# uthree/tinyvc

Measured on AMD Instinct MI355X. Metric: audio-samples/sec (16 kHz) end-to-end VC, higher is better.
Workload: dtype f32 (fp32 in / out / accumulate; channel contractions as two-term fp16 splits on v_mfma_f32_32x32x16_f16: 22-bit significands, three part-products per fp32 product)

## Files before the change

tinyvc_amd/csrc/knn.hip:

```cpp
#include "knn_blob.h"
#include "knn_search.h"
#include "split_fp16.h"
#include "tvc_common.h"

namespace tvc {

constexpr int KNN_BLOCKS = 1024;

constexpr int QN_WAVES = 16;
static __global__ __launch_bounds__(QN_WAVES * 64) void query_normalize_kernel(const float* __restrict__ src, float* __restrict__ qn, int B, int Bsrc, int T,
                                                                     uint4* __restrict__ qh, int* __restrict__ cnt, int* __restrict__ flag,
                                                                     const KnnSegs segs, int* __restrict__ col2seg) {
    __shared__ float part[QN_WAVES][64];
    const int lane = threadIdx.x & 63, wave = threadIdx.x >> 6;
    const long ncols = (long)B * T;
    long n, nn;
    bool ok;
    int sg;
    if (qh) {
        const int tile = blockIdx.x >> 2;
        sg = seg_find<3>(segs, tile);
        const KnnSeg g = seg_get(segs, sg);
        const long loc = (long)(tile - g.u[3]) * 256 + (blockIdx.x & 3) * 64 + lane;
        ok = loc < g.ncols;
        n = g.col0 + loc;
        nn = ok ? n : g.col0 + g.ncols - 1;
    } else {
        n = blockIdx.x * 64L + lane;
        ok = n < ncols;
        nn = ok ? n : ncols - 1;
        sg = col2seg ? seg_find<4>(segs, (int)nn) : 0;
    }
    if (blockIdx.x == 0 && flag)
        for (int i = threadIdx.x; i < segs.n; i += QN_WAVES * 64) flag[i] = 0;
    if (wave == 0 && ok && cnt) cnt[n] = 0;
    if (wave == 0 && ok && col2seg) col2seg[n] = sg;
    const int b = (int)(nn / T), t = (int)(nn - (long)b * T);
    const float* p = src + (long)(b % Bsrc) * KD * T + t;
    float* q = qn + (long)b * KD * T + t;
    constexpr int KW = KD / QN_WAVES;
    const int k0 = wave * KW;
    float x[KW];
#pragma unroll
    for (int i = 0; i < KW; ++i) x[i] = p[(long)(k0 + i) * T];
    float s = 0.f;
#pragma unroll
    for (int i = 0; i < KW; ++i) s = fmaf(x[i], x[i], s);
    part[wave][lane] = s;
    __syncthreads();
    float ss = part[0][lane];
#pragma unroll
    for (int w = 1; w < QN_WAVES; ++w) ss += part[w][lane];
    const float den = sqrtf(ss) + 1e-6f;
    uint4* qhp = qh ? qh + (blockIdx.x >> 2) * (long)(STEPS * 2 * 256) + (blockIdx.x & 3) * 64 + lane : nullptr;
#pragma unroll
    for (int i = 0; i < KW; i += 8) {
        const int k = k0 + i;
        float v[8];
#pragma unroll
        for (int j = 0; j < 8; ++j) v[j] = ok ? x[i + j] / den : 0.f;
        if (ok) {
#pragma unroll
            for (int j = 0; j < 8; ++j) q[(long)(k + j) * T] = v[j];
        }
        if (qh) {
            unsigned o[4];
#pragma unroll
            for (int j = 0; j < 4; ++j) {
                const __half2 h = __floats2half2_rn(v[2 * j], v[2 * j + 1]);
                o[j] = (unsigned)__half_as_ushort(__low2half(h)) | ((unsigned)__half_as_ushort(__high2half(h)) << 16);
            }
            qhp[(long)(k >> 3) * 256] = make_uint4(o[0], o[1], o[2], o[3]);
        }
    }
}

typedef __bf16 bf16x8 __attribute__((ext_vector_type(8)));
typedef __bf16 bf16x2 __attribute__((ext_vector_type(2)));
__device__ __forceinline__ void split8_bf3(const float (&v)[8], uint4& p1, uint4& p2, uint4& p3) {
    unsigned o1[4], o2[4], o3[4];
#pragma unroll
    for (int j = 0; j < 4; ++j) {
        f32x2 a = {v[2 * j], v[2 * j + 1]};
        bf16x2 h1 = __builtin_convertvector(a, bf16x2);
        f32x2 r = a - __builtin_convertvector(h1, f32x2);
        bf16x2 h2 = __builtin_convertvector(r, bf16x2);
        f32x2 r2 = r - __builtin_convertvector(h2, f32x2);
        bf16x2 h3 = __builtin_convertvector(r2, bf16x2);
        o1[j] = __builtin_bit_cast(unsigned, h1);
        o2[j] = __builtin_bit_cast(unsigned, h2);
        o3[j] = __builtin_bit_cast(unsigned, h3);
    }
    p1 = make_uint4(o1[0], o1[1], o1[2], o1[3]);
    p2 = make_uint4(o2[0], o2[1], o2[2], o2[3]);
    p3 = make_uint4(o3[0], o3[1], o3[2], o3[3]);
}
__device__ __forceinline__ void split8_half(const u32x4 h8, uint4& p1, uint4& p2) {
    const f16x8 hv = __builtin_bit_cast(f16x8, h8);
    unsigned o1[4], o2[4];
#pragma unroll
    for (int j = 0; j < 4; ++j) {
        f32x2 a = {(float)hv[2 * j], (float)hv[2 * j + 1]};
        bf16x2 h1 = __builtin_convertvector(a, bf16x2);
        f32x2 r = a - __builtin_convertvector(h1, f32x2);
        bf16x2 h2 = __builtin_convertvector(r, bf16x2);
        o1[j] = __builtin_bit_cast(unsigned, h1);
        o2[j] = __builtin_bit_cast(unsigned, h2);
    }
    p1 = make_uint4(o1[0], o1[1], o1[2], o1[3]);
    p2 = make_uint4(o2[0], o2[1], o2[2], o2[3]);
}

constexpr int KNN_QT = 256;
constexpr int KNN_A_U4 = 12 * 64, KNN_X_U4 = 3 * 2 * KNN_QT;
template <bool F16>
__device__ __forceinline__ void knn_topk_body(const float* __restrict__ blob, long Npad, int N, const float* __restrict__ qn, int ncols, int col0, int cstride,
                                              int T, int unit, int nsplit, int tiles_per_split, float* __restrict__ cand_v, int* __restrict__ cand_i,
                                              uint4* smem) {
    constexpr int NP = F16 ? 2 : 3;
    constexpr int GP = F16 ? 4 : 12;
    uint4* As = smem;
    uint4* Xs = smem + 2 * KNN_A_U4;
    const uint4* img = F16 ? blob_img16(blob, KIND_F16, N, Npad) : blob_img3(blob, N);
    const float* inv = blob_inv(blob, KIND_F16, N, Npad);

    const int tid = threadIdx.x, lane = tid & 63, wave = tid >> 6;
    const int wm = wave >> 2, wn = wave & 3;
    const int l31 = lane & 31, lh = lane >> 5;
    const int split = unit % nsplit;
    const int qtile = unit / nsplit;
    const int n0 = qtile * KNN_QT;
    const int mtiles = (int)(Npad >> 7);
    const int mt_lo = split * tiles_per_split;
    const int mt_hi = min(mtiles, mt_lo + tiles_per_split);
    const int G = (mt_hi - mt_lo) * STEPS;

    const float* qp;
    int xdst;
    {
        const int g = tid >> 8, pos = tid & 255;
        int n = n0 + pos;
        n = col0 + (n < ncols ? n : ncols - 1);
        const int b = n / T, t = n - b * T;
        qp = qn + ((long)b * KD + 8 * g) * T + t;
        xdst = g * KNN_QT + pos;
    }
    const bool a2 = !F16 && wave < 4;
    const bool a1 = !F16 || wave < 4;
    float xr[8];
    u32x4 ar[2];
    auto gload = [&](int g) __attribute__((always_inline)) {
        const int mt = mt_lo + g / STEPS, st = g - (g / STEPS) * STEPS;
        const uint4* src = img + ((long)mt * STEPS + st) * (GP * 64) + lane;
        if (a1) ar[0] = *reinterpret_cast<const u32x4*>(src + wave * 64);
        if (a2) ar[1] = *reinterpret_cast<const u32x4*>(src + (wave + 8) * 64);
#pragma unroll
        for (int j = 0; j < 8; ++j) xr[j] = qp[(long)(st * 16 + j) * T];
    };
    auto lstore = [&](int buf) __attribute__((always_inline)) {
        uint4* ab = As + buf * KNN_A_U4;
        if (F16) {
            if (a1) {
                uint4 p1, p2;
                split8_half(ar[0], p1, p2);
                ab[(wave * 2) * 64 + lane] = p1;
                ab[(wave * 2 + 1) * 64 + lane] = p2;
            }
        } else {
            *reinterpret_cast<u32x4*>(ab + wave * 64 + lane) = ar[0];
            if (a2) *reinterpret_cast<u32x4*>(ab + (wave + 8) * 64 + lane) = ar[1];
        }
        uint4 p1, p2, p3;
        split8_bf3(xr, p1, p2, p3);
        uint4* xb = Xs + buf * KNN_X_U4;
        xb[xdst] = p1;
        xb[2 * KNN_QT + xdst] = p2;
        xb[4 * KNN_QT + xdst] = p3;
    };

    Top4 top[2];
    top[0].init();
    top[1].init();
    f32x16 acc[2][2];
#pragma unroll
    for (int i = 0; i < 2; ++i)
#pragma unroll
        for (int j = 0; j < 2; ++j)
#pragma unroll
            for (int r = 0; r < 16; ++r) acc[i][j][r] = 0.f;

    if (G > 0) {
        gload(0);
        lstore(0);
        if (G > 1) gload(1);
        slab_barrier();
    }
    for (int g = 0; g < G; ++g) {
        const int cur = g & 1;
        if (g + 1 < G) {
            lstore(cur ^ 1);
            if (g + 2 < G) gload(g + 2);
        }
        const uint4* as = As + cur * KNN_A_U4 + wm * (2 * NP * 64) + lane;
        const uint4* xs = Xs + cur * KNN_X_U4 + lh * KNN_QT + wn * 64 + l31;
        bf16x8 af[2][NP], bf[2][3];
#pragma unroll
        for (int j = 0; j < 2; ++j)
#pragma unroll
            for (int p = 0; p < 3; ++p) bf[j][p] = __builtin_bit_cast(bf16x8, xs[p * 2 * KNN_QT + j * 32]);
#pragma unroll
        for (int i = 0; i < 2; ++i)
#pragma unroll
            for (int p = 0; p < NP; ++p) af[i][p] = __builtin_bit_cast(bf16x8, as[(i * NP + p) * 64]);
        constexpr int NQ = F16 ? 5 : 6;
        constexpr int PA3[6] = {2, 1, 0, 1, 0, 0}, PB3[6] = {0, 1, 2, 0, 1, 0};
        constexpr int PA2[5] = {1, 0, 1, 0, 0}, PB2[5] = {1, 2, 0, 1, 0};
#pragma unroll
        for (int q = 0; q < NQ; ++q)
#pragma unroll
            for (int i = 0; i < 2; ++i)
#pragma unroll
                for (int j = 0; j < 2; ++j)
                    acc[i][j] = __builtin_amdgcn_mfma_f32_32x32x16_bf16(af[i][F16 ? PA2[q < 5 ? q : 0] : PA3[q]], bf[j][F16 ? PB2[q < 5 ? q : 0] : PB3[q]],
                                                                        acc[i][j], 0, 0, 0);
        const int st = g - (g / STEPS) * STEPS;
        if (st == STEPS - 1) {
            const int m0 = (mt_lo + g / STEPS) * 128;
#pragma unroll
            for (int i = 0; i < 2; ++i)
#pragma unroll
                for (int r = 0; r < 16; ++r) {
                    const int row = m0 + (wm * 2 + i) * 32 + (r & 3) + 8 * (r >> 2) + 4 * lh;
                    if (row < N) {
                        const float sc = F16 ? inv[row] : 1.f;
#pragma unroll
                        for (int j = 0; j < 2; ++j) top[j].insert(nan_max(F16 ? acc[i][j][r] * sc : acc[i][j][r]), row);
                    }
#pragma unroll
                    for (int j = 0; j < 2; ++j) acc[i][j][r] = 0.f;
                }
        }
        slab_barrier();
    }

    float (*mv)[16] = reinterpret_cast<float (*)[16]>(smem);
    int (*mi)[16] = reinterpret_cast<int (*)[16]>(reinterpret_cast<float*>(smem) + KNN_QT * 16);
#pragma unroll
    for (int j = 0; j < 2; ++j) {
        const int q = wn * 64 + j * 32 + l31;
        const int slot = (wm * 2 + lh) * 4;
#pragma unroll
        for (int e = 0; e < 4; ++e) {
            mv[q][slot + e] = top[j].v[e];
            mi[q][slot + e] = top[j].i[e];
        }
    }
    __syncthreads();
    if (tid < KNN_QT) {
        Top4 t4;
        t4.init();
        for (int e = 0; e < 16; ++e) t4.insert(mv[tid][e], mi[tid][e]);
        int n = n0 + tid;
        if (n < ncols) {
            long o = ((long)split * cstride + col0 + n) * 4;
#pragma unroll
            for (int e = 0; e < 4; ++e) {
                cand_v[o + e] = t4.v[e];
                cand_i[o + e] = t4.i[e];
            }
        }
    }
}

static __global__ __launch_bounds__(512) void knn_topk_split_kernel(const KnnSegs segs, const float* __restrict__ qn, int cstride, int T,
                                                                    float* __restrict__ cand_v, int* __restrict__ cand_i,
                                                                    const int* __restrict__ flags) {
    __shared__ __attribute__((aligned(16))) uint4 smem[2 * (KNN_A_U4 + KNN_X_U4)];
    const int si = seg_find<2>(segs, blockIdx.x);
    const KnnSeg g = seg_get(segs, si);
    if (g.two && flags[si] == 0) return;
    const int kind = blob_kind(g.blob);
    const int unit = blockIdx.x - g.u[2];
    if (kind == KIND_F16) knn_topk_body<true>(g.blob, blob_npad(g.N), g.N, qn, g.ncols, g.col0, cstride, T, unit, g.nsE, g.tpsE, cand_v, cand_i, smem);
    else knn_topk_body<false>(g.blob, blob_npad(g.N), g.N, qn, g.ncols, g.col0, cstride, T, unit, g.nsE, g.tpsE, cand_v, cand_i, smem);
}

constexpr int C_QT = 256, C_MT = 256, C_K = 64, C_STEPS = KD / C_K;
constexpr int C_A_U4 = 4 * 8 * 64, C_X_U4 = 4 * 2 * C_QT;
constexpr int C_LDS = 2 * (C_A_U4 + C_X_U4) * 16;
constexpr int C_CAP = 256;
constexpr float C_EPS = 1.25e-3f;
constexpr int KNN_COARSE_MIN = 4096;

struct Top4V {
    float v[4];
    __device__ __forceinline__ void init() { v[0] = v[1] = v[2] = v[3] = -INFINITY; }
    __device__ __forceinline__ void insert(float x) {
        if (!(x > v[3])) return;
        if (x > v[0]) { v[3] = v[2]; v[2] = v[1]; v[1] = v[0]; v[0] = x; }
        else if (x > v[1]) { v[3] = v[2]; v[2] = v[1]; v[1] = x; }
        else if (x > v[2]) { v[3] = v[2]; v[2] = x; }
        else v[3] = x;
    }
};

template <bool F16, int MODE>
static __device__ __forceinline__ void knn_coarse_body(const float* __restrict__ blob, long Npad, int N, const uint4* __restrict__ qh,
                                                       int ncols, int cstride, int unit, int nsplit, int tiles_per_split, int t2_cover,
                                                       float* __restrict__ c4v, int ns_sample,
                                                       int* __restrict__ cnt, int* __restrict__ cand, float* __restrict__ candv,
                                                       int* __restrict__ overflow) {
    extern __shared__ __attribute__((aligned(16))) uint4 csmem[];
    uint4* As = csmem;
    uint4* Xs = csmem + 2 * C_A_U4;
    const int kind = F16 ? KIND_F16 : KIND_F32;
    const uint4* img = blob_img16(blob, kind, N, Npad);
    const float* inv = blob_inv(blob, kind, N, Npad);

    const int tid = threadIdx.x, lane = tid & 63, wave = tid >> 6;
    const int wm = wave >> 2, wn = wave & 3;
    const int l31 = lane & 31, lh = lane >> 5;
    const int split = unit % nsplit;
    const int qtile = unit / nsplit;
    const int n0 = qtile * C_QT;
    const int mtiles = (int)(Npad >> 7);
    const int t_lo = split * tiles_per_split;
    const int t_hi = min(t2_cover, t_lo + tiles_per_split);
    const int G = (t_hi - t_lo) * C_STEPS;

    const uint4* xsrc = qh + (long)qtile * (STEPS * 2 * 256) + (tid & 511);
    u32x4 ar[4], xr[4];
    auto gload = [&](int g) __attribute__((always_inline)) {
        const int t2 = t_lo + g / C_STEPS, st = g - (g / C_STEPS) * C_STEPS;
#pragma unroll
        for (int i = 0; i < 4; ++i) {
            const int piece = wave + 8 * i, k16 = piece >> 3, mt8 = piece & 7;
            int t128 = 2 * t2 + (mt8 >> 2);
            t128 = t128 < mtiles ? t128 : mtiles - 1;
            ar[i] = *reinterpret_cast<const u32x4*>(img + (((long)t128 * STEPS + 4 * st + k16) * 4 + (mt8 & 3)) * 64 + lane);
            xr[i] = *reinterpret_cast<const u32x4*>(xsrc + (long)(4 * st + i) * 512);
        }
    };
    auto lstore = [&](int buf) __attribute__((always_inline)) {
#pragma unroll
        for (int i = 0; i < 4; ++i) {
            *reinterpret_cast<u32x4*>(As + buf * C_A_U4 + tid + 512 * i) = ar[i];
            *reinterpret_cast<u32x4*>(Xs + buf * C_X_U4 + tid + 512 * i) = xr[i];
        }
    };

    Top4V top[2];
    top[0].init();
    top[1].init();
    float th[2] = {INFINITY, INFINITY};
    if (MODE == 1) {
#pragma unroll
        for (int j = 0; j < 2; ++j) {
            const int n = n0 + wn * 64 + j * 32 + l31;
            if (n < ncols) {
                Top4V t4;
                t4.init();
                for (int sp = 0; sp < ns_sample; ++sp) {
                    const float4 v4 = *reinterpret_cast<const float4*>(c4v + ((long)sp * cstride + n) * 4);
                    t4.insert(v4.x);
                    t4.insert(v4.y);
                    t4.insert(v4.z);
                    t4.insert(v4.w);
                }
                th[j] = t4.v[3] - 2.f * C_EPS;
            }
        }
    }
    f32x16 acc[4][2];
#pragma unroll
    for (int i = 0; i < 4; ++i)
#pragma unroll
        for (int j = 0; j < 2; ++j)
#pragma unroll
            for (int r = 0; r < 16; ++r) acc[i][j][r] = 0.f;

    if (G > 0) {
        gload(0);
        lstore(0);
        gload(G > 1 ? 1 : 0);
        slab_barrier();
    }
    for (int g = 0; g < G; ++g) {
        const int cur = g & 1;
        lstore(cur ^ 1);
        gload(g + 2 < G ? g + 2 : G - 1);
        const uint4* as = As + cur * C_A_U4 + wm * (4 * 64) + lane;
        const uint4* xs = Xs + cur * C_X_U4 + lh * C_QT + wn * 64 + l31;
#pragma unroll
        for (int k16 = 0; k16 < 4; ++k16) {
            f16x8 af[4], bf[2];
#pragma unroll
            for (int i = 0; i < 4; ++i) af[i] = __builtin_bit_cast(f16x8, as[(k16 * 8 + i) * 64]);
#pragma unroll
            for (int j = 0; j < 2; ++j) bf[j] = __builtin_bit_cast(f16x8, xs[k16 * 2 * C_QT + j * 32]);
#pragma unroll
            for (int i = 0; i < 4; ++i)
#pragma unroll
                for (int j = 0; j < 2; ++j) acc[i][j] = __builtin_amdgcn_mfma_f32_32x32x16_f16(af[i], bf[j], acc[i][j], 0, 0, 0);
        }
        const int st = g - (g / C_STEPS) * C_STEPS;
        if (st == C_STEPS - 1) {
            const int t2 = t_lo + g / C_STEPS;
            const int m0 = t2 * C_MT;
            float imx = 1.f;
            if (F16) {
                const float* im = blob_invmax(blob, Npad);
                const int ta = 2 * t2 < mtiles ? 2 * t2 : mtiles - 1, tb = 2 * t2 + 1 < mtiles ? 2 * t2 + 1 : mtiles - 1;
                imx = fmaxf(im[ta], im[tb]);
            }
            const bool whole = m0 + C_MT <= N;
#pragma unroll
            for (int i = 0; i < 4; ++i)
#pragma unroll
                for (int j = 0; j < 2; ++j) {
                    float mx = acc[i][j][0];
                    bool anynan = false;
#pragma unroll
                    for (int r = 1; r < 16; ++r) mx = fmaxf(mx, acc[i][j][r]);
#pragma unroll
                    for (int r = 0; r < 16; ++r) anynan |= acc[i][j][r] != acc[i][j][r];
                    bool maybe;
                    if (MODE == 0) maybe = anynan || !((F16 ? fmaxf(mx, 0.f) * imx : mx) <= top[j].v[3]);
                    else maybe = anynan || (F16 ? fmaxf(mx, 0.f) * imx : mx) >= th[j];
                    if (__builtin_amdgcn_ballot_w64(maybe) != 0ull) {
#pragma unroll
                        for (int r = 0; r < 16; ++r) {
                            const int row = m0 + (wm * 4 + i) * 32 + (r & 3) + 8 * (r >> 2) + 4 * lh;
                            if (whole || row < N) {
                                const float a = acc[i][j][r];
                                if (MODE == 0) {
                                    if (!F16) {
                                        top[j].insert(nan_max(a));
                                    } else if (!(fmaxf(a, 0.f) * imx <= top[j].v[3])) {
                                        top[j].insert(nan_max(a * inv[row]));
                                    }
                                } else {
                                    bool hit;
                                    float cv = a;
                                    if (!F16) hit = !(a < th[j]);
                                    else {
                                        hit = a != a || (fmaxf(a, 0.f) * imx >= th[j]);
                                        if (hit) {
                                            cv = a * inv[row];
                                            hit = a != a || cv >= th[j];
                                        }
                                    }
                                    hit = hit && th[j] != INFINITY;
                                    if (hit) {
                                        const int n = n0 + wn * 64 + j * 32 + l31;
                                        const int pos = atomicAdd(&cnt[n], 1);
                                        if (pos < C_CAP) {
                                            cand[(long)n * C_CAP + pos] = row;
                                            candv[(long)n * C_CAP + pos] = cv;
                                        } else *overflow = 1;
                                    }
                                }
                            }
                        }
                    }
#pragma unroll
                    for (int r = 0; r < 16; ++r) acc[i][j][r] = 0.f;
                }
        }
        slab_barrier();
    }
    if (MODE == 1) return;

    float (*mv)[16] = reinterpret_cast<float (*)[16]>(csmem);
#pragma unroll
    for (int j = 0; j < 2; ++j) {
        const int q = wn * 64 + j * 32 + l31;
        const int slot = (wm * 2 + lh) * 4;
#pragma unroll
        for (int e = 0; e < 4; ++e) mv[q][slot + e] = top[j].v[e];
    }
    __syncthreads();
    if (tid < C_QT) {
        Top4V t4;
        t4.init();
        for (int e = 0; e < 16; ++e) t4.insert(mv[tid][e]);
        const int n = n0 + tid;
        if (n < ncols) {
            const long o = ((long)split * cstride + n) * 4;
#pragma unroll
            for (int e = 0; e < 4; ++e) c4v[o + e] = t4.v[e];
        }
    }
}

template <int MODE>
static __global__ __launch_bounds__(512) void knn_coarse_kernel(const KnnSegs segs, const uint4* __restrict__ qh, int cstride,
                                                                float* __restrict__ c4v, int* __restrict__ cnt, int* __restrict__ cand,
                                                                float* __restrict__ candv, int* __restrict__ flags) {
    const int si = seg_find<MODE>(segs, blockIdx.x);
    const KnnSeg g = seg_get(segs, si);
    const int unit = blockIdx.x - g.u[MODE];
    const int nsplit = MODE ? g.nsB : g.nsA, tps = MODE ? g.tpsB : g.tpsA, cover = MODE ? g.t2 : g.sample;
    const uint4* q = qh + (long)g.u[3] * (STEPS * 2 * 256);
    float* c4 = c4v + (long)g.col0 * 4;
    int* ct = cnt + g.col0;
    int* cd = cand + (long)g.col0 * C_CAP;
    float* cdv = candv + (long)g.col0 * C_CAP;
    if (blob_kind(g.blob) == KIND_F16)
        knn_coarse_body<true, MODE>(g.blob, blob_npad(g.N), g.N, q, g.ncols, cstride, unit, nsplit, tps, cover, c4, g.nsA, ct, cd, cdv, flags + si);
    else
        knn_coarse_body<false, MODE>(g.blob, blob_npad(g.N), g.N, q, g.ncols, cstride, unit, nsplit, tps, cover, c4, g.nsA, ct, cd, cdv, flags + si);
}

static __global__ __launch_bounds__(256) void knn_rescore_kernel(const KnnSegs segs, const int* __restrict__ col2seg, const float* __restrict__ qn,
                                                                 int ncols, int T, const int* __restrict__ cnt, const int* __restrict__ cand,
                                                                 const float* __restrict__ candv, float* __restrict__ rv, int* __restrict__ ri) {
    constexpr int RG = 4;
    const int lane = threadIdx.x & 63;
    const int n = blockIdx.x * 4 + (threadIdx.x >> 6);
    if (n >= ncols) return;
    const KnnSeg g = seg_get(segs, col2seg ? __builtin_amdgcn_readfirstlane(col2seg[n]) : 0);
    if (!g.two) return;
    const float* __restrict__ blob = g.blob;
    const int N = g.N;
    const long Npad = blob_npad(g.N);
    const int kind = blob_kind(blob);
    const float* inv = blob_inv(blob, kind, N, Npad);
    const int b = n / T, t = n - b * T;
    const float* qp = qn + (long)b * KD * T + t;
    int rowl[C_CAP / 64];
    float cvl[C_CAP / 64];
#pragma unroll
    for (int c = 0; c < C_CAP / 64; ++c) {
        rowl[c] = cand[(long)n * C_CAP + 64 * c + lane];
        cvl[c] = candv[(long)n * C_CAP + 64 * c + lane];
    }
    const int nc = min(cnt[n], C_CAP);
    Top4 t4;
    t4.init();
    float th2;
    {
        float rk[C_CAP / 64];
#pragma unroll
        for (int c = 0; c < C_CAP / 64; ++c) {
            if (!(64 * c + lane < nc)) {
                cvl[c] = -INFINITY;
                rowl[c] = 0;
            }
            rk[c] = cvl[c] == cvl[c] ? cvl[c] : -INFINITY;
        }
        float wm = -INFINITY;
#pragma unroll
        for (int round = 0; round < 4; ++round) {
            float lm = rk[0];
#pragma unroll
            for (int c = 1; c < C_CAP / 64; ++c) lm = fmaxf(lm, rk[c]);
            wm = lm;
#pragma unroll
            for (int o = 32; o > 0; o >>= 1) wm = fmaxf(wm, __shfl_xor(wm, o));
            const unsigned long long who = __builtin_amdgcn_ballot_w64(lm == wm);
            if (lane == __builtin_ctzll(who)) {
                bool done = false;
#pragma unroll
                for (int c = 0; c < C_CAP / 64; ++c)
                    if (!done && rk[c] == wm) {
                        rk[c] = -INFINITY;
                        done = true;
                    }
            }
        }
        th2 = wm - 2.f * C_EPS;
    }
    static_assert(C_CAP == 256, "four 64-entry chunks");
    if (kind == KIND_F16) {
        const uint4* img = blob_img16(blob, kind, N, Npad);
        float qs[2][8];
#pragma unroll
        for (int h = 0; h < 2; ++h)
#pragma unroll
            for (int j = 0; j < 8; ++j) {
                const int seg = lane + 64 * h;
                qs[h][j] = seg < 96 ? qp[(long)(8 * seg + j) * T] : 0.f;
            }
        for (int base = 0, ch = 0; base < nc; base += 64, ++ch) {
            const int mine = ch == 0 ? rowl[0] : (ch == 1 ? rowl[1] : (ch == 2 ? rowl[2] : rowl[3]));
            const float cvv = ch == 0 ? cvl[0] : (ch == 1 ? cvl[1] : (ch == 2 ? cvl[2] : cvl[3]));
            unsigned long long mask = __builtin_amdgcn_ballot_w64(base + lane < nc && !(cvv < th2));
            while (mask) {
                int row[RG];
                bool live[RG];
                float d[RG], iv[RG];
                u32x4 w[RG][2];
                int pos = 0;
#pragma unroll
                for (int g = 0; g < RG; ++g) {
                    live[g] = mask != 0ull;
                    if (live[g]) {
                        pos = __builtin_ctzll(mask);
                        mask &= mask - 1;
                    }
                    row[g] = __shfl(mine, pos);
                    const long rbase = ((long)(row[g] >> 7) * STEPS * 4 + ((row[g] & 127) >> 5)) * 64 + (row[g] & 31);
#pragma unroll
                    for (int h = 0; h < 2; ++h) {
                        const int seg = lane + 64 * h < 96 ? lane + 64 * h : 0;
                        w[g][h] = *reinterpret_cast<const u32x4*>(img + rbase + (long)(seg >> 1) * 256 + (seg & 1) * 32);
                    }
                    iv[g] = inv[row[g]];
                }
#pragma unroll
                for (int g = 0; g < RG; ++g) {
                    d[g] = 0.f;
#pragma unroll
                    for (int h = 0; h < 2; ++h) {
                        if (lane + 64 * h < 96) {
                            const f16x8 hv = __builtin_bit_cast(f16x8, w[g][h]);
#pragma unroll
                            for (int j = 0; j < 8; ++j) d[g] = fmaf(qs[h][j], (float)hv[j], d[g]);
                        }
                    }
                }
#pragma unroll
                for (int o = 32; o > 0; o >>= 1)
#pragma unroll
                    for (int g = 0; g < RG; ++g) d[g] += __shfl_xor(d[g], o);
#pragma unroll
                for (int g = 0; g < RG; ++g)
                    if (live[g]) t4.insert(nan_max(d[g] * iv[g]), row[g]);
            }
        }
    } else {
        float qv[12];
#pragma unroll
        for (int u = 0; u < 12; ++u) qv[u] = qp[(long)(lane + 64 * u) * T];
        const float* rows = blob_rows(blob);
        for (int base = 0, ch = 0; base < nc; base += 64, ++ch) {
            const int mine = ch == 0 ? rowl[0] : (ch == 1 ? rowl[1] : (ch == 2 ? rowl[2] : rowl[3]));
            const float cvv = ch == 0 ? cvl[0] : (ch == 1 ? cvl[1] : (ch == 2 ? cvl[2] : cvl[3]));
            unsigned long long mask = __builtin_amdgcn_ballot_w64(base + lane < nc && !(cvv < th2));
            while (mask) {
                int row[RG];
                bool live[RG];
                float d[RG], iv[RG], xv[RG][12];
                int pos = 0;
#pragma unroll
                for (int g = 0; g < RG; ++g) {
                    live[g] = mask != 0ull;
                    if (live[g]) {
                        pos = __builtin_ctzll(mask);
                        mask &= mask - 1;
                    }
                    row[g] = __shfl(mine, pos);
                    const float* rp = rows + (long)row[g] * KD + lane;
#pragma unroll
                    for (int u = 0; u < 12; ++u) xv[g][u] = rp[64 * u];
                    iv[g] = inv[row[g]];
                }
#pragma unroll
                for (int g = 0; g < RG; ++g) {
                    d[g] = 0.f;
#pragma unroll
                    for (int u = 0; u < 12; ++u) d[g] = fmaf(qv[u], xv[g][u], d[g]);
                }
#pragma unroll
                for (int o = 32; o > 0; o >>= 1)
#pragma unroll
                    for (int g = 0; g < RG; ++g) d[g] += __shfl_xor(d[g], o);
#pragma unroll
                for (int g = 0; g < RG; ++g)
                    if (live[g]) t4.insert(nan_max(d[g] * iv[g]), row[g]);
            }
        }
    }
    if (nc < 4) {
#pragma unroll
        for (int e = 0; e < 4; ++e) {
            t4.v[e] = INFINITY;
            t4.i[e] = e;
        }
    }
    if (lane == 0) {
#pragma unroll
        for (int e = 0; e < 4; ++e) {
            rv[(long)n * 4 + e] = t4.v[e];
            ri[(long)n * 4 + e] = t4.i[e];
        }
    }
}

static void split_plan(int blocks, int qtiles, int cover, int* ns, int* tps) {
    int n = (blocks + qtiles - 1) / qtiles;
    if (n > cover) n = cover;
    if (n < 1) n = 1;
    *tps = (cover + n - 1) / n;
    *ns = (cover + *tps - 1) / *tps;
}

int knn_call_plan(tvc_ctx* ctx, const KnnSegIn* in, int nin, int ncols, KnnCall* c) {
    static_assert(KNN_QT == C_QT, "one query tiling for both searches");
    c->ncols = ncols;
    for (int i = 0; i < nin; ++i) {
        if (in[i].N > 0x7fffff00L) return fail(ctx, TVC_ERR_ARG, "index too large");
        if (in[i].ncols <= 0) continue;
        if (!c->seg.empty() && c->seg.back().blob == in[i].blob && c->seg.back().col0 + c->seg.back().ncols == in[i].col0) {
            c->seg.back().ncols += in[i].ncols;
            continue;
        }
        KnnSeg g{};
        g.blob = in[i].blob;
        g.N = (int)in[i].N;
        g.col0 = in[i].col0;
        g.ncols = in[i].ncols;
        c->seg.push_back(g);
    }
    if (c->seg.empty()) return fail(ctx, TVC_ERR_ARG, "knn: no query columns");
    for (auto& g : c->seg) c->cq += (g.ncols + C_QT - 1) / C_QT;
    int mt_max = 1;
    int tile = 0;
    for (auto& g : c->seg) {
        const long Npad = blob_npad(g.N);
        const int mtiles = (int)(Npad / 128);
        const int qt = (g.ncols + C_QT - 1) / C_QT;
        mt_max = mtiles > mt_max ? mtiles : mt_max;
        g.two = g.N >= KNN_COARSE_MIN;
        g.t2 = (int)((Npad + C_MT - 1) / C_MT);
        g.sample = g.t2 / 8 < 5 ? 5 : g.t2 / 8;
        if (g.sample > g.t2) g.sample = g.t2;
        split_plan(768, c->cq, g.sample, &g.nsA, &g.tpsA);
        split_plan(768, c->cq, g.t2, &g.nsB, &g.tpsB);
        split_plan(KNN_BLOCKS, c->cq, mtiles, &g.nsE, &g.tpsE);
        g.u[0] = c->units[0];
        g.u[1] = c->units[1];
        g.u[2] = c->units[2];
        g.u[3] = tile;
        if (g.two) {
            c->units[0] += qt * g.nsA;
            c->units[1] += qt * g.nsB;
            c->two = true;
        }
        c->units[2] += qt * g.nsE;
        tile += qt;
    }
    if (c->seg.size() == 1) c->ns_cv = c->seg[0].nsE;
    else {
        const int cq_min = (ncols + C_QT - 1) / C_QT;
        c->ns_cv = (KNN_BLOCKS + cq_min - 1) / cq_min;
        c->ns_cv = c->ns_cv < mt_max ? c->ns_cv : mt_max;
    }
    return 0;
}

template <int MODE>
static int coarse_launch(tvc_ctx* ctx, hipStream_t s, const KnnCall& c, const KnnLists& L, const uint4* qh, float* c4v, int* cnt, int* cand, float* candv) {
    TVC_CHECK(lds_optin<knn_coarse_kernel<MODE>>(ctx, C_LDS, "knn coarse"));
    hipLaunchKernelGGL((knn_coarse_kernel<MODE>), dim3((unsigned)c.units[MODE]), dim3(512), C_LDS, s, L.segs, qh, c.ncols, c4v, cnt, cand, candv, L.flag);
    return 0;
}

static int coarse_max_nsplit(int qtiles) { return (768 + qtiles - 1) / qtiles; }

int knn_candidates(tvc_ctx* ctx, hipStream_t s, Ws& ws, const float* src, const KnnCall& c, int B, int T, KnnLists* L, int Bsrc) {
    const int nseg = (int)c.seg.size();
    float* qn = ws.get<float>((size_t)B * KD * T);
    L->cv = ws.get<float>((size_t)c.ns_cv * c.ncols * 4);
    L->ci = ws.get<int>((size_t)c.ns_cv * c.ncols * 4);
    int* dtab = nseg > 1 ? ws.get<int>((size_t)nseg * sizeof(KnnSeg) / sizeof(int)) : nullptr;
    L->col2seg = nseg > 1 ? ws.get<int>((size_t)c.ncols) : nullptr;
    uint4* qh = nullptr;
    float* c4v = nullptr;
    int *cnt = nullptr, *cand = nullptr;
    float* candv = nullptr;
    if (c.two) {
        qh = ws.get<uint4>((size_t)c.cq * STEPS * 2 * 256);
        c4v = ws.get<float>((size_t)coarse_max_nsplit((c.ncols + C_QT - 1) / C_QT) * c.ncols * 4);
        cnt = ws.get<int>((size_t)c.ncols);
        cand = ws.get<int>((size_t)c.ncols * C_CAP);
        candv = ws.get<float>((size_t)c.ncols * C_CAP);
        L->rv = ws.get<float>((size_t)c.ncols * 4);
        L->ri = ws.get<int>((size_t)c.ncols * 4);
        L->flag = ws.get<int>((size_t)(nseg > 64 ? nseg : 64));
    }
    if (ws.dry) return 0;
    L->segs.n = nseg;
    L->segs.one = c.seg[0];
    L->segs.d = reinterpret_cast<const KnnSeg*>(dtab);
    if (dtab) {
        std::vector<int> words((size_t)nseg * sizeof(KnnSeg) / sizeof(int));
        std::memcpy(words.data(), c.seg.data(), words.size() * sizeof(int));
        TVC_CHECK(upload_ints(ctx, s, words, dtab));
    }
    const int nblk = c.two ? c.cq * 4 : (c.ncols + 63) / 64;
    hipLaunchKernelGGL(query_normalize_kernel, dim3(nblk), dim3(QN_WAVES * 64), 0, s, src, qn, B, Bsrc > 0 ? Bsrc : B, T, qh, cnt, L->flag, L->segs, L->col2seg);
    if (c.two) {
        ProfScope ps(ctx, s, ws, "knn.coarse+rescore");
        TVC_CHECK((coarse_launch<0>(ctx, s, c, *L, qh, c4v, cnt, cand, candv)));
        TVC_CHECK((coarse_launch<1>(ctx, s, c, *L, qh, c4v, cnt, cand, candv)));
        hipLaunchKernelGGL(knn_rescore_kernel, dim3((c.ncols + 3) / 4), dim3(256), 0, s, L->segs, (const int*)L->col2seg, qn, c.ncols, T, cnt, cand, candv, L->rv, L->ri);
    }
    ProfScope ps(ctx, s, ws, "knn.exact");
    hipLaunchKernelGGL(knn_topk_split_kernel, dim3((unsigned)c.units[2]), dim3(512), 0, s, L->segs, qn, c.ncols, T, L->cv, L->ci, (const int*)L->flag);
    return 0;
}

}
```

tinyvc_amd/csrc/knn_search.h:

```cpp
#pragma once
#include "tvc_common.h"

namespace tvc {

struct KnnSeg {
    const float* blob;
    int N, col0, ncols;
    int two;
    int sample, t2;
    int nsA, tpsA, nsB, tpsB;
    int nsE, tpsE;
    int u[4];
};
static_assert(sizeof(KnnSeg) % sizeof(int) == 0, "uploaded as ints");
struct KnnSegs {
    const KnnSeg* d;
    int n;
    KnnSeg one;
};
template <int F>
__device__ __forceinline__ int seg_find(const KnnSegs& S, int v) {
    if (S.n == 1) return 0;
    int lo = 0, hi = S.n - 1;
    while (lo < hi) {
        const int mid = (lo + hi + 1) >> 1;
        const int key = F == 4 ? S.d[mid].col0 : S.d[mid].u[F];
        if (key <= v) lo = mid;
        else hi = mid - 1;
    }
    return lo;
}
__device__ __forceinline__ KnnSeg seg_get(const KnnSegs& S, int i) {
    KnnSeg g;
    const bool one = S.n == 1;
    const KnnSeg* __restrict__ d = S.d + (one ? 0 : i);
#define TVC_SEG_FIELD(f) g.f = one ? S.one.f : d->f
    TVC_SEG_FIELD(blob);
    TVC_SEG_FIELD(N);
    TVC_SEG_FIELD(col0);
    TVC_SEG_FIELD(ncols);
    TVC_SEG_FIELD(two);
    TVC_SEG_FIELD(sample);
    TVC_SEG_FIELD(t2);
    TVC_SEG_FIELD(nsA);
    TVC_SEG_FIELD(tpsA);
    TVC_SEG_FIELD(nsB);
    TVC_SEG_FIELD(tpsB);
    TVC_SEG_FIELD(nsE);
    TVC_SEG_FIELD(tpsE);
    TVC_SEG_FIELD(u[0]);
    TVC_SEG_FIELD(u[1]);
    TVC_SEG_FIELD(u[2]);
    TVC_SEG_FIELD(u[3]);
#undef TVC_SEG_FIELD
    return g;
}

__device__ __forceinline__ float nan_max(float x) { return x != x ? INFINITY : x; }

struct Top4 {
    float v[4];
    int i[4];
    __device__ __forceinline__ void init() {
#pragma unroll
        for (int j = 0; j < 4; ++j) {
            v[j] = -INFINITY;
            i[j] = 0x7fffffff;
        }
    }
    __device__ __forceinline__ static bool better(float a, int ia, float b, int ib) { return a > b || (a == b && ia < ib); }
    __device__ __forceinline__ void insert(float x, int ix) {
        if (!better(x, ix, v[3], i[3])) return;
        if (better(x, ix, v[0], i[0])) { v[3] = v[2]; i[3] = i[2]; v[2] = v[1]; i[2] = i[1]; v[1] = v[0]; i[1] = i[0]; v[0] = x; i[0] = ix; }
        else if (better(x, ix, v[1], i[1])) { v[3] = v[2]; i[3] = i[2]; v[2] = v[1]; i[2] = i[1]; v[1] = x; i[1] = ix; }
        else if (better(x, ix, v[2], i[2])) { v[3] = v[2]; i[3] = i[2]; v[2] = x; i[2] = ix; }
        else { v[3] = x; i[3] = ix; }
    }
};

struct KnnCall {
    std::vector<KnnSeg> seg;
    int ncols = 0, cq = 0;
    int units[3] = {0, 0, 0};
    int ns_cv = 1;
    bool two = false;
};

struct KnnLists {
    float* cv = nullptr;
    int* ci = nullptr;
    float* rv = nullptr;
    int* ri = nullptr;
    int* flag = nullptr;
    int* col2seg = nullptr;
    KnnSegs segs{};
};

int knn_call_plan(tvc_ctx* ctx, const KnnSegIn* in, int nin, int ncols, KnnCall* c);
int knn_candidates(tvc_ctx* ctx, hipStream_t s, Ws& ws, const float* src, const KnnCall& c, int B, int T, KnnLists* L, int Bsrc = 0);

}
```

Baseline: 700.5 million.

## Run coarse kNN pass as persistent walk over (query tile, index tile) pairs

```diff
diff --git a/tinyvc_amd/csrc/knn.hip b/tinyvc_amd/csrc/knn.hip
--- a/tinyvc_amd/csrc/knn.hip
+++ b/tinyvc_amd/csrc/knn.hip
@@ -304,40 +304,167 @@
     }
 };
 
+struct CoarseSeg {
+    int lo, hi;
+    int rows, tiles, wa, ww;
+    int N, ncols, col0, nsA, tpsA, kind, mtiles, qt0, si;
+    const uint4* img;
+    const float *inv, *invmax;
+    template <int MODE>
+    __device__ __forceinline__ void load(const KnnSegs& S, int i) {
+        const KnnSeg g = seg_get(S, i);
+        si = i;
+        N = g.N;
+        ncols = g.ncols;
+        col0 = g.col0;
+        nsA = g.nsA;
+        tpsA = g.tpsA;
+        qt0 = g.u[3];
+        rows = (g.ncols + 255) / 256;
+        tiles = MODE ? g.t2 : g.sample;
+        wa = g.wa;
+        ww = g.ww;
+        lo = g.u[MODE];
+        hi = lo + rows * tiles;
+        kind = blob_kind(g.blob);
+        const long Npad = blob_npad(g.N);
+        mtiles = (int)(Npad >> 7);
+        img = blob_img16(g.blob, kind, g.N, Npad);
+        inv = blob_inv(g.blob, kind, g.N, Npad);
+        invmax = blob_invmax(g.blob, Npad);
+    }
+};
+
 template <bool F16, int MODE>
-static __device__ __forceinline__ void knn_coarse_body(const float* __restrict__ blob, long Npad, int N, const uint4* __restrict__ qh,
-                                                       int ncols, int cstride, int unit, int nsplit, int tiles_per_split, int t2_cover,
-                                                       float* __restrict__ c4v, int ns_sample,
-                                                       int* __restrict__ cnt, int* __restrict__ cand, float* __restrict__ candv,
-                                                       int* __restrict__ overflow) {
+static __device__ __forceinline__ void coarse_tile_end(f32x16 (&acc)[4][2], Top4V (&top)[2], const float (&th)[2], const CoarseSeg& sg, int t2,
+                                                       int n0, int* __restrict__ cnt, int* __restrict__ cand, float* __restrict__ candv,
+                                                       int* __restrict__ overflow, int wm, int wn, int lh, int l31) {
+    const int N = sg.N, mtiles = sg.mtiles;
+    const float* __restrict__ inv = sg.inv;
+    const int m0 = t2 * C_MT;
+    float imx = 1.f;
+    if (F16) {
+        const float* im = sg.invmax;
+        const int ta = 2 * t2 < mtiles ? 2 * t2 : mtiles - 1, tb = 2 * t2 + 1 < mtiles ? 2 * t2 + 1 : mtiles - 1;
+        imx = fmaxf(im[ta], im[tb]);
+    }
+    const bool whole = m0 + C_MT <= N;
+#pragma unroll
+    for (int i = 0; i < 4; ++i)
+#pragma unroll
+        for (int j = 0; j < 2; ++j) {
+            float mx = acc[i][j][0];
+            bool anynan = false;
+#pragma unroll
+            for (int r = 1; r < 16; ++r) mx = fmaxf(mx, acc[i][j][r]);
+#pragma unroll
+            for (int r = 0; r < 16; ++r) anynan |= acc[i][j][r] != acc[i][j][r];
+            bool maybe;
+            if (MODE == 0) maybe = anynan || !((F16 ? fmaxf(mx, 0.f) * imx : mx) <= top[j].v[3]);
+            else maybe = anynan || (F16 ? fmaxf(mx, 0.f) * imx : mx) >= th[j];
+            if (__builtin_amdgcn_ballot_w64(maybe) != 0ull) {
+#pragma unroll
+                for (int r = 0; r < 16; ++r) {
+                    const int row = m0 + (wm * 4 + i) * 32 + (r & 3) + 8 * (r >> 2) + 4 * lh;
+                    if (whole || row < N) {
+                        const float a = acc[i][j][r];
+                        if (MODE == 0) {
+                            if (!F16) {
+                                top[j].insert(nan_max(a));
+                            } else if (!(fmaxf(a, 0.f) * imx <= top[j].v[3])) {
+                                top[j].insert(nan_max(a * inv[row]));
+                            }
+                        } else {
+                            bool hit;
+                            float cv = a;
+                            if (!F16) hit = !(a < th[j]);
+                            else {
+                                hit = a != a || (fmaxf(a, 0.f) * imx >= th[j]);
+                                if (hit) {
+                                    cv = a * inv[row];
+                                    hit = a != a || cv >= th[j];
+                                }
+                            }
+                            hit = hit && th[j] != INFINITY;
+                            if (hit) {
+                                const int n = n0 + wn * 64 + j * 32 + l31;
+                                const int pos = atomicAdd(&cnt[n], 1);
+                                if (pos < C_CAP) {
+                                    cand[(long)n * C_CAP + pos] = row;
+                                    candv[(long)n * C_CAP + pos] = cv;
+                                } else *overflow = 1;
+                            }
+                        }
+                    }
+                }
+            }
+#pragma unroll
+            for (int r = 0; r < 16; ++r) acc[i][j][r] = 0.f;
+        }
+}
+
+template <int MODE, int KIND>
+static __device__ __forceinline__ void knn_coarse_body(const KnnSegs& segs, const uint4* __restrict__ qh, int cstride, int slot, int grid, int pairs,
+                                                       float* __restrict__ c4v, int* __restrict__ cnt, int* __restrict__ cand,
+                                                       float* __restrict__ candv, int* __restrict__ flags) {
     extern __shared__ __attribute__((aligned(16))) uint4 csmem[];
     uint4* As = csmem;
     uint4* Xs = csmem + 2 * C_A_U4;
-    const int kind = F16 ? KIND_F16 : KIND_F32;
-    const uint4* img = blob_img16(blob, kind, N, Npad);
-    const float* inv = blob_inv(blob, kind, N, Npad);
 
     const int tid = threadIdx.x, lane = tid & 63, wave = tid >> 6;
     const int wm = wave >> 2, wn = wave & 3;
     const int l31 = lane & 31, lh = lane >> 5;
-    const int split = unit % nsplit;
-    const int qtile = unit / nsplit;
-    const int n0 = qtile * C_QT;
-    const int mtiles = (int)(Npad >> 7);
-    const int t_lo = split * tiles_per_split;
-    const int t_hi = min(t2_cover, t_lo + tiles_per_split);
-    const int G = (t_hi - t_lo) * C_STEPS;
-
-    const uint4* xsrc = qh + (long)qtile * (STEPS * 2 * 256) + (tid & 511);
+
+    CoarseSeg ls, cs;
+    int p_lo, p_hi, split = 0, q0 = 0;
+    if (MODE == 0) {
+        ls.load<MODE>(segs, seg_find<0>(segs, slot));
+        cs = ls;
+        const int unit = slot - ls.lo;
+        split = unit % ls.nsA;
+        q0 = unit / ls.nsA;
+        p_lo = split * ls.tpsA;
+        p_hi = min(ls.tiles, p_lo + ls.tpsA);
+    } else {
+        long lo, hi;
+        knn_walk_range(pairs, grid, slot, &lo, &hi);
+        p_lo = (int)lo;
+        p_hi = (int)hi;
+        ls.lo = ls.hi = 0;
+        cs.lo = cs.hi = 0;
+    }
+    const int G = (p_hi - p_lo) * C_STEPS;
+    auto locate = [&](CoarseSeg& sg, int p, int& q, int& t) __attribute__((always_inline)) {
+        if (MODE == 0) {
+            q = q0;
+            t = p;
+        } else {
+            if (p < sg.lo || p >= sg.hi) sg.load<MODE>(segs, seg_find<1>(segs, p));
+            knn_walk_pair(p - sg.lo, sg.rows, sg.tiles, sg.wa, sg.ww, &q, &t);
+        }
+    };
+
+    int ld_pr = -1, ld_t2 = 0, ld_st = 0;
+    const uint4* xsrc = qh;
     u32x4 ar[4], xr[4];
-    auto gload = [&](int g) __attribute__((always_inline)) {
-        const int t2 = t_lo + g / C_STEPS, st = g - (g / C_STEPS) * C_STEPS;
+    auto ld_seek = [&](int g) __attribute__((always_inline)) {
+        const int pr = g / C_STEPS;
+        ld_st = g - pr * C_STEPS;
+        if (pr != ld_pr) {
+            ld_pr = pr;
+            int q;
+            locate(ls, p_lo + pr, q, ld_t2);
+            xsrc = qh + (long)(ls.qt0 + q) * (STEPS * 2 * 256) + tid;
+        }
+    };
+    auto gload = [&]() __attribute__((always_inline)) {
+        const int mtiles = ls.mtiles, st = ld_st;
 #pragma unroll
         for (int i = 0; i < 4; ++i) {
             const int piece = wave + 8 * i, k16 = piece >> 3, mt8 = piece & 7;
-            int t128 = 2 * t2 + (mt8 >> 2);
+            int t128 = 2 * ld_t2 + (mt8 >> 2);
             t128 = t128 < mtiles ? t128 : mtiles - 1;
-            ar[i] = *reinterpret_cast<const u32x4*>(img + (((long)t128 * STEPS + 4 * st + k16) * 4 + (mt8 & 3)) * 64 + lane);
+            ar[i] = *reinterpret_cast<const u32x4*>(ls.img + (((long)t128 * STEPS + 4 * st + k16) * 4 + (mt8 & 3)) * 64 + lane);
             xr[i] = *reinterpret_cast<const u32x4*>(xsrc + (long)(4 * st + i) * 512);
         }
     };
@@ -353,24 +480,7 @@
     top[0].init();
     top[1].init();
     float th[2] = {INFINITY, INFINITY};
-    if (MODE == 1) {
-#pragma unroll
-        for (int j = 0; j < 2; ++j) {
-            const int n = n0 + wn * 64 + j * 32 + l31;
-            if (n < ncols) {
-                Top4V t4;
-                t4.init();
-                for (int sp = 0; sp < ns_sample; ++sp) {
-                    const float4 v4 = *reinterpret_cast<const float4*>(c4v + ((long)sp * cstride + n) * 4);
-                    t4.insert(v4.x);
-                    t4.insert(v4.y);
-                    t4.insert(v4.z);
-                    t4.insert(v4.w);
-                }
-                th[j] = t4.v[3] - 2.f * C_EPS;
-            }
-        }
-    }
+    int cq = -1, csi = -1;
     f32x16 acc[4][2];
 #pragma unroll
     for (int i = 0; i < 4; ++i)
@@ -380,15 +490,18 @@
             for (int r = 0; r < 16; ++r) acc[i][j][r] = 0.f;
 
     if (G > 0) {
-        gload(0);
+        ld_seek(0);
+        gload();
         lstore(0);
-        gload(G > 1 ? 1 : 0);
+        ld_seek(G > 1 ? 1 : 0);
+        gload();
         slab_barrier();
+        ld_seek(G > 2 ? 2 : G - 1);
     }
     for (int g = 0; g < G; ++g) {
         const int cur = g & 1;
         lstore(cur ^ 1);
-        gload(g + 2 < G ? g + 2 : G - 1);
+        gload();
         const uint4* as = As + cur * C_A_U4 + wm * (4 * 64) + lane;
         const uint4* xs = Xs + cur * C_X_U4 + lh * C_QT + wn * 64 + l31;
 #pragma unroll
@@ -403,70 +516,39 @@
 #pragma unroll
                 for (int j = 0; j < 2; ++j) acc[i][j] = __builtin_amdgcn_mfma_f32_32x32x16_f16(af[i], bf[j], acc[i][j], 0, 0, 0);
         }
-        const int st = g - (g / C_STEPS) * C_STEPS;
-        if (st == C_STEPS - 1) {
-            const int t2 = t_lo + g / C_STEPS;
-            const int m0 = t2 * C_MT;
-            float imx = 1.f;
-            if (F16) {
-                const float* im = blob_invmax(blob, Npad);
-                const int ta = 2 * t2 < mtiles ? 2 * t2 : mtiles - 1, tb = 2 * t2 + 1 < mtiles ? 2 * t2 + 1 : mtiles - 1;
-                imx = fmaxf(im[ta], im[tb]);
-            }
-            const bool whole = m0 + C_MT <= N;
-#pragma unroll
-            for (int i = 0; i < 4; ++i)
+        const int pr = g / C_STEPS;
+        if (g - pr * C_STEPS == C_STEPS - 1) {
+            int q, t2;
+            locate(cs, p_lo + pr, q, t2);
+            const int n0 = q * C_QT;
+            if (MODE == 1 && (q != cq || cs.si != csi)) {
+                cq = q;
+                csi = cs.si;
 #pragma unroll
                 for (int j = 0; j < 2; ++j) {
-                    float mx = acc[i][j][0];
-                    bool anynan = false;
-#pragma unroll
-                    for (int r = 1; r < 16; ++r) mx = fmaxf(mx, acc[i][j][r]);
-#pragma unroll
-                    for (int r = 0; r < 16; ++r) anynan |= acc[i][j][r] != acc[i][j][r];
-                    bool maybe;
-                    if (MODE == 0) maybe = anynan || !((F16 ? fmaxf(mx, 0.f) * imx : mx) <= top[j].v[3]);
-                    else maybe = anynan || (F16 ? fmaxf(mx, 0.f) * imx : mx) >= th[j];
-                    if (__builtin_amdgcn_ballot_w64(maybe) != 0ull) {
-#pragma unroll
-                        for (int r = 0; r < 16; ++r) {
-                            const int row = m0 + (wm * 4 + i) * 32 + (r & 3) + 8 * (r >> 2) + 4 * lh;
-                            if (whole || row < N) {
-                                const float a = acc[i][j][r];
-                                if (MODE == 0) {
-                                    if (!F16) {
-                                        top[j].insert(nan_max(a));
-                                    } else if (!(fmaxf(a, 0.f) * imx <= top[j].v[3])) {
-                                        top[j].insert(nan_max(a * inv[row]));
-                                    }
-                                } else {
-                                    bool hit;
-                                    float cv = a;
-                                    if (!F16) hit = !(a < th[j]);
-                                    else {
-                                        hit = a != a || (fmaxf(a, 0.f) * imx >= th[j]);
-                                        if (hit) {
-                                            cv = a * inv[row];
-                                            hit = a != a || cv >= th[j];
-                                        }
-                                    }
-                                    hit = hit && th[j] != INFINITY;
-                                    if (hit) {
-                                        const int n = n0 + wn * 64 + j * 32 + l31;
-                                        const int pos = atomicAdd(&cnt[n], 1);
-                                        if (pos < C_CAP) {
-                                            cand[(long)n * C_CAP + pos] = row;
-                                            candv[(long)n * C_CAP + pos] = cv;
-                                        } else *overflow = 1;
-                                    }
-                                }
-                            }
+                    const int n = n0 + wn * 64 + j * 32 + l31;
+                    th[j] = INFINITY;
+                    if (n < cs.ncols) {
+                        Top4V t4;
+                        t4.init();
+                        for (int sp = 0; sp < cs.nsA; ++sp) {
+                            const float4 v4 = *reinterpret_cast<const float4*>(c4v + ((long)sp * cstride + cs.col0 + n) * 4);
+                            t4.insert(v4.x);
+                            t4.insert(v4.y);
+                            t4.insert(v4.z);
+                            t4.insert(v4.w);
                         }
+                        th[j] = t4.v[3] - 2.f * C_EPS;
                     }
-#pragma unroll
-                    for (int r = 0; r < 16; ++r) acc[i][j][r] = 0.f;
                 }
-        }
+            }
+            int* ct = cnt + cs.col0;
+            int* cd = cand + (long)cs.col0 * C_CAP;
+            float* cdv = candv + (long)cs.col0 * C_CAP;
+            if (KIND == KIND_F16 || (KIND == 2 && cs.kind == KIND_F16)) coarse_tile_end<true, MODE>(acc, top, th, cs, t2, n0, ct, cd, cdv, flags + cs.si, wm, wn, lh, l31);
+            else coarse_tile_end<false, MODE>(acc, top, th, cs, t2, n0, ct, cd, cdv, flags + cs.si, wm, wn, lh, l31);
+        }
+        ld_seek(g + 3 < G ? g + 3 : G - 1);
         slab_barrier();
     }
     if (MODE == 1) return;
@@ -475,18 +557,18 @@
 #pragma unroll
     for (int j = 0; j < 2; ++j) {
         const int q = wn * 64 + j * 32 + l31;
-        const int slot = (wm * 2 + lh) * 4;
-#pragma unroll
-        for (int e = 0; e < 4; ++e) mv[q][slot + e] = top[j].v[e];
+        const int slot4 = (wm * 2 + lh) * 4;
+#pragma unroll
+        for (int e = 0; e < 4; ++e) mv[q][slot4 + e] = top[j].v[e];
     }
     __syncthreads();
     if (tid < C_QT) {
         Top4V t4;
         t4.init();
         for (int e = 0; e < 16; ++e) t4.insert(mv[tid][e]);
-        const int n = n0 + tid;
-        if (n < ncols) {
-            const long o = ((long)split * cstride + n) * 4;
+        const int n = q0 * C_QT + tid;
+        if (n < cs.ncols) {
+            const long o = ((long)split * cstride + cs.col0 + n) * 4;
 #pragma unroll
             for (int e = 0; e < 4; ++e) c4v[o + e] = t4.v[e];
         }
@@ -494,22 +576,13 @@
 }
 
 template <int MODE>
-static __global__ __launch_bounds__(512) void knn_coarse_kernel(const KnnSegs segs, const uint4* __restrict__ qh, int cstride,
+static __global__ __launch_bounds__(512) void knn_coarse_kernel(const KnnSegs segs, const uint4* __restrict__ qh, int cstride, int pairs,
                                                                 float* __restrict__ c4v, int* __restrict__ cnt, int* __restrict__ cand,
                                                                 float* __restrict__ candv, int* __restrict__ flags) {
-    const int si = seg_find<MODE>(segs, blockIdx.x);
-    const KnnSeg g = seg_get(segs, si);
-    const int unit = blockIdx.x - g.u[MODE];
-    const int nsplit = MODE ? g.nsB : g.nsA, tps = MODE ? g.tpsB : g.tpsA, cover = MODE ? g.t2 : g.sample;
-    const uint4* q = qh + (long)g.u[3] * (STEPS * 2 * 256);
-    float* c4 = c4v + (long)g.col0 * 4;
-    int* ct = cnt + g.col0;
-    int* cd = cand + (long)g.col0 * C_CAP;
-    float* cdv = candv + (long)g.col0 * C_CAP;
-    if (blob_kind(g.blob) == KIND_F16)
-        knn_coarse_body<true, MODE>(g.blob, blob_npad(g.N), g.N, q, g.ncols, cstride, unit, nsplit, tps, cover, c4, g.nsA, ct, cd, cdv, flags + si);
-    else
-        knn_coarse_body<false, MODE>(g.blob, blob_npad(g.N), g.N, q, g.ncols, cstride, unit, nsplit, tps, cover, c4, g.nsA, ct, cd, cdv, flags + si);
+    const int slot = knn_walk_slot((int)blockIdx.x, (int)gridDim.x), grid = (int)gridDim.x;
+    if (segs.n > 1) knn_coarse_body<MODE, 2>(segs, qh, cstride, slot, grid, pairs, c4v, cnt, cand, candv, flags);
+    else if (blob_kind(segs.one.blob) == KIND_F16) knn_coarse_body<MODE, KIND_F16>(segs, qh, cstride, slot, grid, pairs, c4v, cnt, cand, candv, flags);
+    else knn_coarse_body<MODE, KIND_F32>(segs, qh, cstride, slot, grid, pairs, c4v, cnt, cand, candv, flags);
 }
 
 static __global__ __launch_bounds__(256) void knn_rescore_kernel(const KnnSegs segs, const int* __restrict__ col2seg, const float* __restrict__ qn,
@@ -727,19 +800,24 @@
         g.sample = g.t2 / 8 < 5 ? 5 : g.t2 / 8;
         if (g.sample > g.t2) g.sample = g.t2;
         split_plan(768, c->cq, g.sample, &g.nsA, &g.tpsA);
-        split_plan(768, c->cq, g.t2, &g.nsB, &g.tpsB);
         split_plan(KNN_BLOCKS, c->cq, mtiles, &g.nsE, &g.tpsE);
         g.u[0] = c->units[0];
         g.u[1] = c->units[1];
         g.u[2] = c->units[2];
         g.u[3] = tile;
         if (g.two) {
+            if ((long)c->units[1] + (long)qt * g.t2 > 0x7fffffffL) return fail(ctx, TVC_ERR_ARG, "knn: too many (query tile, index tile) pairs");
             c->units[0] += qt * g.nsA;
-            c->units[1] += qt * g.nsB;
+            c->units[1] += qt * g.t2;
             c->two = true;
         }
         c->units[2] += qt * g.nsE;
         tile += qt;
+    }
+    if (c->two) {
+        c->gridB = knn_walk_grid(c->units[1], ctx->ncu);
+        for (auto& g : c->seg)
+            if (g.two) knn_walk_shape(c->units[1], c->gridB, (g.ncols + C_QT - 1) / C_QT, g.t2, &g.wa, &g.ww);
     }
     if (c->seg.size() == 1) c->ns_cv = c->seg[0].nsE;
     else {
@@ -753,7 +831,8 @@
 template <int MODE>
 static int coarse_launch(tvc_ctx* ctx, hipStream_t s, const KnnCall& c, const KnnLists& L, const uint4* qh, float* c4v, int* cnt, int* cand, float* candv) {
     TVC_CHECK(lds_optin<knn_coarse_kernel<MODE>>(ctx, C_LDS, "knn coarse"));
-    hipLaunchKernelGGL((knn_coarse_kernel<MODE>), dim3((unsigned)c.units[MODE]), dim3(512), C_LDS, s, L.segs, qh, c.ncols, c4v, cnt, cand, candv, L.flag);
+    const int grid = MODE ? c.gridB : c.units[0];
+    hipLaunchKernelGGL((knn_coarse_kernel<MODE>), dim3((unsigned)grid), dim3(512), C_LDS, s, L.segs, qh, c.ncols, c.units[1], c4v, cnt, cand, candv, L.flag);
     return 0;
 }
 
diff --git a/tinyvc_amd/csrc/knn_search.h b/tinyvc_amd/csrc/knn_search.h
--- a/tinyvc_amd/csrc/knn_search.h
+++ b/tinyvc_amd/csrc/knn_search.h
@@ -1,4 +1,5 @@
 #pragma once
+#include "knn_walk.h"
 #include "tvc_common.h"
 
 namespace tvc {
@@ -8,7 +9,8 @@
     int N, col0, ncols;
     int two;
     int sample, t2;
-    int nsA, tpsA, nsB, tpsB;
+    int nsA, tpsA;
+    int wa, ww;
     int nsE, tpsE;
     int u[4];
 };
@@ -44,8 +46,8 @@
     TVC_SEG_FIELD(t2);
     TVC_SEG_FIELD(nsA);
     TVC_SEG_FIELD(tpsA);
-    TVC_SEG_FIELD(nsB);
-    TVC_SEG_FIELD(tpsB);
+    TVC_SEG_FIELD(wa);
+    TVC_SEG_FIELD(ww);
     TVC_SEG_FIELD(nsE);
     TVC_SEG_FIELD(tpsE);
     TVC_SEG_FIELD(u[0]);
@@ -82,6 +84,7 @@
     std::vector<KnnSeg> seg;
     int ncols = 0, cq = 0;
     int units[3] = {0, 0, 0};
+    int gridB = 0;
     int ns_cv = 1;
     bool two = false;
 };
diff --git a/tinyvc_amd/csrc/knn_walk.h b/tinyvc_amd/csrc/knn_walk.h
--- /dev/null
+++ b/tinyvc_amd/csrc/knn_walk.h
@@ -0,0 +1,50 @@
+#pragma once
+
+#if defined(__HIPCC__)
+#define TVC_WALK_FN __host__ __device__ inline
+#else
+#define TVC_WALK_FN inline
+#endif
+
+namespace tvc {
+
+TVC_WALK_FN int knn_walk_grid(long pairs, int ncu) {
+    int slots = ncu / 8 * 8 > 0 ? ncu / 8 * 8 : ncu;
+    slots = slots < 1 ? 1 : slots;
+    return pairs < slots ? (int)pairs : slots;
+}
+
+TVC_WALK_FN int knn_walk_slot(int b, int grid) {
+    const int x = b & 7, q8 = grid >> 3, r8 = grid & 7;
+    return x * q8 + (x < r8 ? x : r8) + (b >> 3);
+}
+
+TVC_WALK_FN void knn_walk_range(long pairs, int grid, int v, long* lo, long* hi) {
+    const long base = pairs / grid, rem = pairs % grid;
+    *lo = v * base + (v < rem ? v : rem);
+    *hi = *lo + base + (v < rem ? 1 : 0);
+}
+
+TVC_WALK_FN void knn_walk_shape(long pairs, int grid, int rows, int tiles, int* a, int* w) {
+    const int m = grid >= 8 ? grid >> 3 : 1;
+    long ww = (pairs + grid / 2) / grid;
+    ww = ww < 1 ? 1 : (ww > tiles ? tiles : ww);
+    long aa = ((long)m * pairs / grid + tiles / 2) / tiles;
+    aa = aa < 1 ? 1 : (aa > rows ? rows : aa);
+    *a = (int)aa;
+    *w = (int)ww;
+}
+
+TVC_WALK_FN void knn_walk_pair(int o, int rows, int tiles, int a, int w, int* q, int* t) {
+    const int band = o / (a * tiles);
+    o -= band * a * tiles;
+    const int h = rows - band * a < a ? rows - band * a : a;
+    const int j = o / (h * w);
+    o -= j * h * w;
+    const int wj = tiles - j * w < w ? tiles - j * w : w;
+    const int i = o / wj;
+    *q = band * a + i;
+    *t = j * w + (o - i * wj);
+}
+
+}
```

Measured after the change: 708.6 million, median of 6. Within noise of the previous version (+1.2%).
